# bravo1goingdark/ucfp

Measured on AMD Instinct MI355X. Metric: fingerprints/sec (batched ingest), higher is better.
Workload: dtype u8; 1 GPU; image multi (pHash+dHash+aHash bundle, 536 B/frame), 100000 synthetic 512x512 GRAY8 frames per GPU resident in HBM (BASELINE.json configs[1]); frames_per_gpu=100000, width=512, height=512, pixfmt=gray8, algorithm=multi

## Files before the change

ucfp_amd/csrc/common.h:

```cpp
#pragma once
#include <hip/hip_runtime.h>
#include <stddef.h>
#include <stdint.h>

#include "../../include/ucfp_hip.h"

namespace ucfp {

int capi_fail(int code, const char* fmt, ...);
int ctx_device(const ucfp_ctx* ctx);
bool have_gfx950();

}

#define HIP_TRY(expr)                                                                                \
    do {                                                                                             \
        hipError_t e_ = (expr);                                                                      \
        if (e_ != hipSuccess)                                                                        \
            return ucfp::capi_fail(UCFP_E_INDEX, "%s failed: %s", #expr, hipGetErrorString(e_));     \
    } while (0)

namespace ucfp {

struct DevArr {
// ... 94 lines not shown
int launch_png_decode(const uint8_t* png, const uint64_t* offsets, size_t n, uint32_t w, uint32_t h, int pixfmt, uint8_t* ws,
                      const PngWs& l, uint8_t* frames, size_t row_stride, size_t frame_stride, int32_t* status,
                      hipStream_t stream, hipStream_t side = nullptr, hipEvent_t fork = nullptr, hipEvent_t join = nullptr);
int launch_png_merge_status(const uint8_t* ws, const PngWs& l, size_t n, uint8_t* out, uint32_t rec, int32_t* status,
                            hipStream_t stream, const UpItem* d_items = nullptr);
size_t png_ragged_ws_bytes(size_t n, size_t png_bytes, size_t raw_total, PngWs* ws);
size_t png_raw_bytes(uint32_t w, uint32_t h, int pixfmt);
int launch_png_decode_ragged(const uint8_t* png, const uint64_t* offsets, const UpItem* d_items, size_t n, const uint32_t max_w[3],
                             uint8_t* ws, const PngWs& l, uint8_t* frames, int32_t* status, hipStream_t stream);

struct JpegWs {
    size_t clean = 0, info = 0, seg = 0, qtab = 0, coef = 0, coef_stride = 0, total = 0;
    size_t jpg_bytes = 0;
    uint32_t bxp = 0, byp = 0, max_seg = 0;
};
size_t jpeg_ws_bytes(size_t n, size_t jpg_bytes, uint32_t w, uint32_t h, JpegWs* ws);
int launch_jpeg_decode(const uint8_t* jpg, const uint64_t* offsets, size_t n, uint32_t w, uint32_t h, uint8_t* ws,
                       const JpegWs& l, uint8_t* frames, size_t row_stride, size_t frame_stride, int32_t* status,
                       hipStream_t stream);
int launch_jpeg_merge_status(const uint8_t* ws, const JpegWs& l, size_t n, uint8_t* out, uint32_t rec, int32_t* status,
                             hipStream_t stream, const UpItem* d_items = nullptr);
void jpeg_plane_geometry(uint32_t w, uint32_t h, uint32_t* bxp, uint32_t* byp, uint32_t* max_seg);
size_t jpeg_ragged_ws_bytes(size_t n, size_t jpg_bytes, size_t seg_words, size_t coef_words, JpegWs* ws);
int launch_jpeg_decode_ragged(const uint8_t* jpg, const uint64_t* offsets, const UpItem* d_items, size_t n, const uint32_t* d_first,
                              size_t idct_groups, uint8_t* ws, const JpegWs& l, uint8_t* frames, int32_t* status, hipStream_t stream);

struct HammingPlan {
    uint32_t qgroups = 0;
    int cap = 24;
    size_t sample_n = 0;
    uint32_t sample_parts = 0;
    size_t per_part = 0;
    size_t robust_n = 0;
    uint32_t slices = 0;
    size_t per_slice = 0;
    bool bound = false;
    size_t bound_n = 0;
    bool fast = false;
    uint32_t nstages = 0;
    size_t stage_end[12] = {0};
    uint32_t cand_cap = 0;
    uint32_t log_cap = 0;
    uint32_t fb_slices = 0;
    size_t fb_per_slice = 0;
};
constexpr uint32_t kHammingMaxBatch = 4096;
HammingPlan hamming_plan(size_t n, uint32_t nq, uint32_t k);
size_t hamming_workspace_bytes(const HammingPlan& p, uint32_t nq, uint32_t k);
int launch_hamming_search(const uint64_t* codes, const uint64_t* ids, size_t n,
                          const uint64_t* queries, uint32_t nq, uint32_t k, uint8_t* ws,
                          const HammingPlan& p, uint64_t* out_ids, uint32_t* out_dist,
                          float* out_scores, uint32_t* out_cnt, hipStream_t stream,
                          const uint32_t* ids_ascending = nullptr);
int launch_ids_order_update(const uint64_t* ids, size_t n, bool first, uint32_t* state, hipStream_t stream);
int launch_hamming_scores(const uint32_t* dist, size_t total, float* scores, hipStream_t stream);

constexpr uint32_t kHammingDirectMaxQ = 8, kHammingDirectMaxK = 32, kHammingDirectZeroBytes = 12288;
bool hamming_direct_ok(size_t n, uint32_t nq, uint32_t k);
size_t hamming_direct_state_bytes();
int launch_hamming_direct(const uint64_t* codes, const uint64_t* ids, size_t n, const uint64_t* queries, uint32_t nq,
                          uint32_t k, uint8_t* state, uint64_t* out_ids, uint32_t* out_dist, float* out_scores,
                          uint32_t* out_cnt, hipStream_t stream, const uint32_t* ids_ascending = nullptr);

struct SelectPlan {
    uint32_t slices = 0;
    size_t per_slice = 0;
};
SelectPlan select_plan(size_t n, uint32_t nq);
bool select_pruned_ok(size_t n, uint32_t nq, uint32_t k);
size_t select_pruned_ws_bytes(size_t n, uint32_t nq);
int launch_select_pruned_u32(const uint32_t* keys, const uint64_t* ids, size_t n, uint32_t nq, uint32_t k, uint32_t* mins,
                             uint64_t* out_ids, uint32_t* out_key, uint32_t* out_cnt, hipStream_t stream,
                             const uint32_t* run_flag);
int launch_select_topk_u32(const uint32_t* keys, const uint64_t* ids, size_t n, const SelectPlan& p,
                           uint32_t nq, uint32_t k, uint64_t* part_ids, uint32_t* part_key,
                           uint32_t* part_cnt, hipStream_t stream, const uint32_t* run_flag = nullptr);
int launch_topk_select_lists_u32(const uint64_t* base_ids, const uint32_t* base_key, const uint32_t* ckey,
                                 const uint32_t* crow, const uint32_t* ccnt, uint32_t cap, const uint64_t* ids,
                                 uint32_t nq, uint32_t k, uint64_t* out_ids, uint32_t* out_key, uint32_t* out_cnt,
                                 uint32_t* overflow, hipStream_t stream);
struct CosinePrunePlan {
    uint32_t cs_shift = 5;
    uint32_t qpad = 16;
    uint32_t nchunks = 0;
    uint32_t waves = 0;
    uint32_t capq = 32;
};
constexpr uint32_t kPruneCand = 2048;
bool cosine_prune_ok(const float* rows, uint32_t dim, const float* queries, uint32_t nq_pass, size_t n, uint32_t k);
CosinePrunePlan cosine_prune_plan(size_t n, uint32_t nq_pass, uint32_t k, bool approx = false);
float cosine_mins_eps(uint32_t dim);
uint32_t cosine_list_queries(uint32_t dim);
bool cosine_mins_f16_ok(const float* rows, uint32_t dim, const float* queries, uint32_t nq_pass, size_t n, uint32_t k);
int launch_cosine_norms_image(const float* queries, size_t nq, uint32_t dim, float* norms, void* image, uint32_t* zero2,
                              hipStream_t stream);
int launch_cosine_mins_f16(const float* rows, const float* norms, size_t n, uint32_t dim, const void* image, const float* qnorm,
                           uint32_t nq_pass, const CosinePrunePlan& p, uint32_t* mins, uint32_t* wmin, uint32_t* flag,
                           hipStream_t stream);
int launch_cosine_keys_dense_mfma(const float* rows, const float* norms, size_t n, uint32_t dim, const float* queries,
                                  const float* qnorm, uint32_t nq_pass, uint32_t* keys, const uint32_t* run_flag,
                                  hipStream_t stream);
int launch_cosine_keys_mins(const float* rows, const float* norms, size_t n, uint32_t dim, const float* queries,
                            const float* qnorm, uint32_t nq_pass, const CosinePrunePlan& p, uint32_t* mins, uint32_t* wmin,
                            hipStream_t stream);
int launch_cosine_keys_list(const float* rows, const float* norms, size_t n, uint32_t dim, const float* queries,
                            const float* qnorm, uint32_t nq_pass, const CosinePrunePlan& p, const void* list,
                            const uint32_t* nlist, uint32_t* ckeys, const uint32_t* fallback_flag, hipStream_t stream);
// ... 191 lines not shown
```

ucfp_amd/csrc/hamming.hip:

```cpp

#include <hip/hip_runtime.h>
#include <math.h>
#include <stdint.h>
#include <stdlib.h>

#include "common.h"

namespace ucfp {

constexpr int kWave = 64;
constexpr uint32_t kSub = 8;

__device__ __forceinline__ uint32_t hamming64(uint64_t q, uint64_t x) {
    const uint32_t lo = (uint32_t)q ^ (uint32_t)x;
    const uint32_t hi = (uint32_t)(q >> 32) ^ (uint32_t)(x >> 32);
    return __builtin_popcount(hi) + __builtin_popcount(lo);
}

__global__ __launch_bounds__(256) void hamming_sample_hist(const uint64_t* __restrict__ codes,
                                                           size_t sample_n, size_t per_part,
                                                           const uint64_t* __restrict__ queries,
                                                           uint32_t nq, uint32_t* __restrict__ hist) {
    __shared__ uint32_t h[65 * kWave];
    const int lane = threadIdx.x & 63, wave = threadIdx.x >> 6;
// ... 982 lines not shown
                bi = oi;
            }
        }
        if (bd == 0xffffffffu) break;
        if (lane == 0) {
            out_ids[(size_t)q * k + r] = bi;
            out_d[(size_t)q * k + r] = bd;
        }
        ld = bd;
        li = bi;
        first = false;
        emitted++;
    }
    if (lane == 0) {
        for (uint32_t r = emitted; r < k; r++) {
            out_ids[(size_t)q * k + r] = ~0ull;
            out_d[(size_t)q * k + r] = 0xffffffffu;
        }
        out_cnt[q] = emitted;
    }
}

__global__ void hamming_reset_lists(uint32_t nq, uint32_t* __restrict__ cand_cnt, uint32_t* __restrict__ overflow) {
    const uint32_t q = blockIdx.x * blockDim.x + threadIdx.x;
    if (q == 0) *overflow = 0;
    if (q < nq)
        for (uint32_t u = 0; u < kSub; u++) cand_cnt[(size_t)q * kSub + u] = 0;
}

__global__ void hamming_scores(const uint32_t* __restrict__ dist, size_t total, float* __restrict__ scores) {
    const size_t i = (size_t)blockIdx.x * blockDim.x + threadIdx.x;
    if (i < total) {
        const uint32_t d = dist[i];
        scores[i] = d == 0xffffffffu ? -1.0f : 1.0f - (float)d * (1.0f / 64.0f);
    }
}


namespace {
void slice_range(size_t n, uint32_t qgroups, uint32_t want_waves, size_t min_per_slice, uint32_t& slices,
                 size_t& per_slice) {
    uint32_t s = (want_waves + qgroups - 1) / (qgroups ? qgroups : 1);
    const size_t max_s = (n + min_per_slice - 1) / min_per_slice;
    if (s > max_s) s = (uint32_t)(max_s ? max_s : 1);
    if (s < 1) s = 1;
    if (s > 8192) s = 8192;
    per_slice = (n + s - 1) / s;
    per_slice = (per_slice + 31) & ~(size_t)31;
    slices = (uint32_t)((n + per_slice - 1) / (per_slice ? per_slice : 1));
    if (slices < 1) slices = 1;
}
}

__global__ void ids_order_update_kernel(const uint64_t* __restrict__ ids, size_t n, bool first, uint32_t* __restrict__ state) {
    const size_t i = (size_t)blockIdx.x * blockDim.x + threadIdx.x;
    if (i >= n) return;
    uint64_t* last = reinterpret_cast<uint64_t*>(state + 2);
    bool ok;
    if (i == 0) ok = first || ids[0] > *last;
    else ok = ids[i] > ids[i - 1];
    if (!ok) state[0] = 0;
}
__global__ void ids_order_last_kernel(const uint64_t* __restrict__ ids, size_t n, uint32_t* __restrict__ state) {
    *reinterpret_cast<uint64_t*>(state + 2) = ids[n - 1];
}
int launch_ids_order_update(const uint64_t* ids, size_t n, bool first, uint32_t* state, hipStream_t stream) {
    if (n == 0) return 0;
    hipLaunchKernelGGL(ids_order_update_kernel, dim3((unsigned)((n + 255) / 256)), dim3(256), 0, stream, ids, n, first, state);
    hipLaunchKernelGGL(ids_order_last_kernel, dim3(1), dim3(1), 0, stream, ids, n, state);
    return 0;
}

static bool few_queries(size_t n, uint32_t nq);
constexpr uint32_t kBoundGroups = 256;
constexpr size_t kBoundCodes = (size_t)1 << 18;

HammingPlan hamming_plan(size_t n, uint32_t nq, uint32_t k) {
    HammingPlan p;
    p.qgroups = (nq + kWave - 1) / kWave;
    p.cap = k <= 16 ? 24 : k <= 40 ? 64 : 160;
    if (n == 0) return p;
    size_t s = 32768;
    if (s > n) s = n;
    p.sample_n = s;
    p.sample_parts = (uint32_t)((s + 1023) / 1024);
    p.per_part = (s + p.sample_parts - 1) / p.sample_parts;
    p.fast = n >= (size_t)1 << 18 && n - 1 <= 0xfffffff0u;
    p.robust_n = n;
    p.bound = p.fast && !few_queries(n, nq) && k <= 64 && !getenv("UCFP_HAMMING_NO_BOUND");
    const bool short_chain = p.bound && nq <= 256 && k <= 16;
    if (p.bound) {
        size_t bc = short_chain ? (size_t)1 << 20 : kBoundCodes;
        static const char* bl = getenv("UCFP_HAMMING_BOUND_LOG2_SMALL");
        if (bl && nq <= 256) bc = (size_t)1 << atoi(bl);
        static const char* bg = getenv("UCFP_HAMMING_BOUND_LOG2_LARGE");
        if (bg && nq > 256) bc = (size_t)1 << atoi(bg);
        p.bound_n = (n < bc ? n : bc) & ~(size_t)(128 - 1);
    }
    if (p.fast) {
        size_t e = p.bound ? p.bound_n : p.sample_n;
        size_t growth = short_chain ? 64 : nq <= 256 ? 8 : 4;
        static const char* gs = getenv("UCFP_HAMMING_GROWTH_SMALL");
        if (gs && nq <= 256) growth = (size_t)atoi(gs);
        static const char* gl = getenv("UCFP_HAMMING_GROWTH_LARGE");
        if (gl && nq > 256) growth = (size_t)atoi(gl);
        static const char* nomerge = getenv("UCFP_HAMMING_NO_STAGE_MERGE");
        do {
            e = e * growth < n ? e * growth : n;
            if (!nomerge && n - e < e / 4) e = n;
            p.stage_end[p.nstages++] = e;
        } while (e < n && p.nstages < 12);
        p.stage_end[p.nstages - 1] = n;
        p.robust_n = 0;
        size_t cc = (size_t)k * growth * 5 * p.nstages * 2;
        if (cc < 2048) cc = 2048;
        if (cc > 65536) cc = 65536;
        cc = (cc + 63) & ~(size_t)63;
        p.cand_cap = (uint32_t)cc;
        p.log_cap = 1024;
        slice_range(n, p.qgroups, 256 * 16, 4096, p.fb_slices, p.fb_per_slice);
        return p;
    }
// ... 175 lines not shown
```

ucfp_amd/csrc/index.hip:

```cpp

#include <hip/hip_runtime.h>

#include <cstdarg>
#include <cstdio>
#include <cstdlib>
#include <cstring>
#include <map>
#include <mutex>
#include <new>
#include <unordered_map>
#include <vector>

#include "../../include/ucfp_hip.h"
#include "common.h"

using ucfp::capi_fail;

namespace {

struct DevBuf {
    uint8_t* p = nullptr;
    size_t cap = 0;
    int ensure(size_t need) {
        if (cap >= need) return 0;
        if (p) (void)hipFree(p);
        p = nullptr;
        cap = 0;
        const size_t want = need + need / 4 + 4096;
        HIP_TRY(hipMalloc((void**)&p, want));
        cap = want;
        return 0;
    }
    void release() {
        if (p) (void)hipFree(p);
        p = nullptr;
        cap = 0;
    }
};

struct Shard {
    uint64_t* ids = nullptr;
    uint8_t* rows = nullptr;
    float* norms = nullptr;
    size_t n = 0, cap = 0;
    std::unordered_map<uint64_t, size_t> pos;
    std::vector<uint64_t> host_ids;
    uint32_t* order = nullptr;
};

__global__ void scatter_rows_kernel(const uint64_t* __restrict__ src_ids, const uint8_t* __restrict__ src_rows,
                                    const uint64_t* __restrict__ dst_row, size_t n, size_t row_bytes,
                                    uint64_t* __restrict__ ids, uint8_t* __restrict__ rows) {
    const size_t i = blockIdx.x;
    if (i >= n) return;
    const size_t r = dst_row[i];
    if (threadIdx.x == 0) ids[r] = src_ids[i];
    const uint32_t* s = reinterpret_cast<const uint32_t*>(src_rows + i * row_bytes);
    uint32_t* d = reinterpret_cast<uint32_t*>(rows + r * row_bytes);
    for (size_t w = threadIdx.x; w < row_bytes / 4; w += blockDim.x) d[w] = s[w];
}

__global__ void gather_norms_kernel(const float* __restrict__ src, const uint64_t* __restrict__ dst_row, size_t n,
                                    float* __restrict__ norms) {
    const size_t i = (size_t)blockIdx.x * blockDim.x + threadIdx.x;
    if (i < n) norms[dst_row[i]] = src[i];
}

int ensure_order_state(Shard& s, hipStream_t st) {
    if (s.order) return 0;
    if (hipMalloc((void**)&s.order, 16) != hipSuccess) return -1;
    static const uint32_t init[4] = {1u, 0u, 0u, 0u};
    if (hipMemcpyAsync(s.order, init, 16, hipMemcpyHostToDevice, st) != hipSuccess) return -1;
    return 0;
}

}

struct ucfp_index {
    ucfp_ctx* ctx = nullptr;
    int device = 0;
    int kind = 0;
    uint32_t dim = 0;
    uint32_t flags = 0;
    size_t row_bytes = 0;
    std::mutex mu;
    std::map<uint32_t, Shard> shards;
    hipStream_t stream = nullptr;
    DevBuf ws_slot[2];
    DevBuf direct_state[2];
    hipEvent_t ws_done[2] = {nullptr, nullptr};
    unsigned ws_next = 0, ws_cur = 0;
    hipEvent_t data_ready = nullptr;
    DevBuf stage;
};

namespace ucfp {
int index_kind(const ucfp_index* ix) { return ix->kind; }
int index_device(const ucfp_index* ix) { return ix->device; }
uint32_t index_dim(const ucfp_index* ix) { return ix->dim; }
}

namespace {

int shard_reserve(ucfp_index* ix, Shard& s, size_t need, hipStream_t st) {
    if (need <= s.cap) return 0;
    size_t ncap = s.cap ? s.cap * 2 : 1024;
    while (ncap < need) ncap *= 2;
    uint64_t* nids = nullptr;
    uint8_t* nrows = nullptr;
    float* nnorms = nullptr;
    HIP_TRY(hipMalloc((void**)&nids, ncap * 8));
    HIP_TRY(hipMalloc((void**)&nrows, ncap * ix->row_bytes));
    if (ix->kind == UCFP_INDEX_COSINE_F32) HIP_TRY(hipMalloc((void**)&nnorms, ncap * 4));
    if (s.n) {
        HIP_TRY(hipMemcpyAsync(nids, s.ids, s.n * 8, hipMemcpyDeviceToDevice, st));
        HIP_TRY(hipMemcpyAsync(nrows, s.rows, s.n * ix->row_bytes, hipMemcpyDeviceToDevice, st));
        if (nnorms) HIP_TRY(hipMemcpyAsync(nnorms, s.norms, s.n * 4, hipMemcpyDeviceToDevice, st));
    }
    HIP_TRY(hipStreamSynchronize(st));
    if (s.ids) (void)hipFree(s.ids);
    if (s.rows) (void)hipFree(s.rows);
    if (s.norms) (void)hipFree(s.norms);
    s.ids = nids;
    s.rows = nrows;
    s.norms = nnorms;
    s.cap = ncap;
    return 0;
}

size_t align256(size_t x) { return (x + 255) & ~(size_t)255; }

int search_shard_dev(ucfp_index* ix, const Shard* s, const void* d_queries, size_t nq, uint32_t k,
                     uint64_t* d_out_ids, float* d_out_scores, uint32_t* d_out_keys, uint32_t* d_out_cnt,
                     hipStream_t st) {
    const size_t n = s ? s->n : 0;
    if (ix->kind == UCFP_INDEX_HAMMING64 && nq <= ucfp::kHammingDirectMaxQ && ucfp::hamming_direct_ok(n, (uint32_t)nq, k) &&
        !getenv("UCFP_HAMMING_NO_DIRECT")) {
        DevBuf& stt = ix->direct_state[ix->ws_cur];
        if (!stt.p) {
            int rc = stt.ensure(ucfp::hamming_direct_state_bytes());
            if (rc) return rc;
            HIP_TRY(hipMemsetAsync(stt.p, 0, ucfp::kHammingDirectZeroBytes, st));
        }
        uint32_t* keys = d_out_keys;
        if (!keys) {
            int rc = ix->ws_slot[ix->ws_cur].ensure(nq * k * 4 + 256);
            if (rc) return rc;
            keys = reinterpret_cast<uint32_t*>(ix->ws_slot[ix->ws_cur].p);
        }
        ucfp::launch_hamming_direct(reinterpret_cast<const uint64_t*>(s->rows), s->ids, n,
                                    reinterpret_cast<const uint64_t*>(d_queries), (uint32_t)nq, k, stt.p, d_out_ids, keys,
                                    d_out_scores, d_out_cnt, st, s->order);
        HIP_TRY(hipGetLastError());
        return 0;
    }
    if (ix->kind == UCFP_INDEX_HAMMING64) {
        const size_t chunk = nq < ucfp::kHammingMaxBatch ? nq : ucfp::kHammingMaxBatch;
        ucfp::HammingPlan p = ucfp::hamming_plan(n, (uint32_t)chunk, k);
        size_t need = ucfp::hamming_workspace_bytes(p, (uint32_t)chunk, k) + 4096;
        if (nq % chunk) {
            const uint32_t tail = (uint32_t)(nq % chunk);
            const size_t nt = ucfp::hamming_workspace_bytes(ucfp::hamming_plan(n, tail, k), tail, k) + 4096;
            need = nt > need ? nt : need;
        }
        uint32_t* keys = d_out_keys;
        size_t keys_off = 0;
        if (!keys) {
            keys_off = align256(need);
            need = keys_off + nq * k * 4;
        }
        int rc = ix->ws_slot[ix->ws_cur].ensure(need);
        if (rc) return rc;
        if (!keys) keys = reinterpret_cast<uint32_t*>(ix->ws_slot[ix->ws_cur].p + keys_off);
        const uint64_t* dq = reinterpret_cast<const uint64_t*>(d_queries);
        for (size_t c0 = 0; c0 < nq; c0 += chunk) {
            const uint32_t cn = (uint32_t)(nq - c0 < chunk ? nq - c0 : chunk);
            if (cn != chunk) p = ucfp::hamming_plan(n, cn, k);
            ucfp::launch_hamming_search(s ? reinterpret_cast<const uint64_t*>(s->rows) : nullptr, s ? s->ids : nullptr,
                                        n, dq + c0, cn, k, ix->ws_slot[ix->ws_cur].p, p, d_out_ids + c0 * k, keys + c0 * k,
                                        d_out_scores ? d_out_scores + c0 * k : nullptr, d_out_cnt + c0, st,
// ... 226 lines not shown
    HIP_TRY(hipGetLastError());
    return 0;
}

int check_search_args(ucfp_index* ix, const void* q, size_t nq, uint32_t k, const void* ids, const void* cnt) {
    if (!ix) return capi_fail(UCFP_E_INVALID, "index is NULL");
    if (k > UCFP_INDEX_MAX_K) return capi_fail(UCFP_E_INVALID, "k = %u exceeds UCFP_INDEX_MAX_K = %u", k, UCFP_INDEX_MAX_K);
    if (nq && k && (!q || !ids || !cnt)) return capi_fail(UCFP_E_INVALID, "queries/out_ids/out_counts is NULL");
    if (nq > 4000000u) return capi_fail(UCFP_E_INVALID, "query batch %zu too large for one call (max 4 000 000)", nq);
    return 0;
}

}

extern "C" {

int ucfp_index_create(ucfp_ctx* ctx, int kind, uint32_t dim, uint32_t flags, ucfp_index** out) {
    if (!ctx || !out) return capi_fail(UCFP_E_INVALID, "ctx/out is NULL");
    *out = nullptr;
    if (kind != UCFP_INDEX_HAMMING64 && kind != UCFP_INDEX_COSINE_F32)
        return capi_fail(UCFP_E_UNSUPPORTED, "unknown index kind %d", kind);
    if (kind == UCFP_INDEX_COSINE_F32 && (dim == 0 || dim > 65536))
        return capi_fail(UCFP_E_INVALID, "cosine index needs 1 <= dim <= 65536 (got %u)", dim);
    ucfp_index* ix = new (std::nothrow) ucfp_index();
    if (!ix) return capi_fail(UCFP_E_INDEX, "out of host memory");
    ix->ctx = ctx;
    ix->device = ucfp::ctx_device(ctx);
    ix->kind = kind;
    ix->dim = kind == UCFP_INDEX_HAMMING64 ? 1 : dim;
    ix->flags = flags;
    ix->row_bytes = kind == UCFP_INDEX_HAMMING64 ? 8 : (size_t)dim * 4;
    hipError_t e = hipSetDevice(ix->device);
    if (e == hipSuccess) e = hipStreamCreateWithFlags(&ix->stream, hipStreamNonBlocking);
    for (int i = 0; i < 2 && e == hipSuccess; i++) e = hipEventCreateWithFlags(&ix->ws_done[i], hipEventDisableTiming);
    if (e == hipSuccess) e = hipEventCreateWithFlags(&ix->data_ready, hipEventDisableTiming);
    if (e != hipSuccess) {
        delete ix;
        return capi_fail(UCFP_E_INDEX, "index stream creation failed: %s", hipGetErrorString(e));
    }
    *out = ix;
    return UCFP_OK;
}

void ucfp_index_destroy(ucfp_index* ix) {
    if (!ix) return;
    (void)hipSetDevice(ix->device);
    (void)hipDeviceSynchronize();
    for (auto& kv : ix->shards) {
        if (kv.second.ids) (void)hipFree(kv.second.ids);
        if (kv.second.rows) (void)hipFree(kv.second.rows);
        if (kv.second.norms) (void)hipFree(kv.second.norms);
        if (kv.second.order) (void)hipFree(kv.second.order);
    }
    for (auto& w : ix->ws_slot) w.release();
    for (auto& w : ix->direct_state) w.release();
    ix->stage.release();
    if (ix->stream) (void)hipStreamDestroy(ix->stream);
    for (hipEvent_t ev : ix->ws_done)
        if (ev) (void)hipEventDestroy(ev);
    if (ix->data_ready) (void)hipEventDestroy(ix->data_ready);
    delete ix;
}

int ucfp_index_upsert(ucfp_index* ix, uint32_t tenant, const uint64_t* ids, const void* rows, size_t n) {
    if (!ix) return capi_fail(UCFP_E_INVALID, "index is NULL");
    if (n == 0) return UCFP_OK;
    if (!ids || !rows) return capi_fail(UCFP_E_INVALID, "ids/rows is NULL");
    std::lock_guard<std::mutex> lk(ix->mu);
    HIP_TRY(hipSetDevice(ix->device));
    Shard& s = ix->shards[tenant];
    hipStream_t st = ix->stream;
    for (hipEvent_t ev : ix->ws_done) HIP_TRY(hipStreamWaitEvent(st, ev, 0));
    HIP_TRY(hipStreamWaitEvent(st, ix->data_ready, 0));
    const bool mapped = !(ix->flags & UCFP_INDEX_APPEND_ONLY);
    std::vector<uint64_t> dst(n);
    std::vector<uint8_t> keep(n, 1);
    size_t new_n = s.n;
    if (mapped) {
        std::unordered_map<uint64_t, size_t> last;
        last.reserve(n * 2);
        for (size_t i = 0; i < n; i++) last[ids[i]] = i;
        for (size_t i = 0; i < n; i++) {
            if (last[ids[i]] != i) {
                keep[i] = 0;
                continue;
            }
            auto it = s.pos.find(ids[i]);
            if (it != s.pos.end()) dst[i] = it->second;
            else dst[i] = new_n++;
        }
    } else {
        for (size_t i = 0; i < n; i++) dst[i] = new_n++;
    }
    int rc = shard_reserve(ix, s, new_n, st);
    if (rc) return rc;
    size_t m = 0;
    for (size_t i = 0; i < n; i++) m += keep[i];
    const size_t o_ids = 0, o_dst = align256(m * 8), o_rows = align256(o_dst + m * 8);
    const size_t o_norm = align256(o_rows + m * ix->row_bytes);
    rc = ix->stage.ensure(o_norm + m * 4 + 256);
    if (rc) return rc;
    std::vector<uint64_t> h_ids(m), h_dst(m);
    std::vector<uint8_t> h_rows(m * ix->row_bytes);
    size_t j = 0;
    for (size_t i = 0; i < n; i++) {
        if (!keep[i]) continue;
        h_ids[j] = ids[i];
        h_dst[j] = dst[i];
        memcpy(h_rows.data() + j * ix->row_bytes, (const uint8_t*)rows + i * ix->row_bytes, ix->row_bytes);
        j++;
    }
    uint8_t* sp = ix->stage.p;
    HIP_TRY(hipMemcpyAsync(sp + o_ids, h_ids.data(), m * 8, hipMemcpyHostToDevice, st));
    HIP_TRY(hipMemcpyAsync(sp + o_dst, h_dst.data(), m * 8, hipMemcpyHostToDevice, st));
    HIP_TRY(hipMemcpyAsync(sp + o_rows, h_rows.data(), m * ix->row_bytes, hipMemcpyHostToDevice, st));
    hipLaunchKernelGGL(scatter_rows_kernel, dim3((unsigned)m), dim3(64), 0, st,
                       reinterpret_cast<const uint64_t*>(sp + o_ids), sp + o_rows,
                       reinterpret_cast<const uint64_t*>(sp + o_dst), m, ix->row_bytes, s.ids, s.rows);
    if (ix->kind == UCFP_INDEX_COSINE_F32) {
        ucfp::launch_cosine_norms(reinterpret_cast<const float*>(sp + o_rows), m, ix->dim,
                                  reinterpret_cast<float*>(sp + o_norm), st);
        hipLaunchKernelGGL(gather_norms_kernel, dim3((unsigned)((m + 255) / 256)), dim3(256), 0, st,
                           reinterpret_cast<const float*>(sp + o_norm), reinterpret_cast<const uint64_t*>(sp + o_dst),
                           m, s.norms);
    }
    if (!mapped && ix->kind == UCFP_INDEX_HAMMING64 && m) {
        if (ensure_order_state(s, st)) return capi_fail(UCFP_E_INDEX, "out of device memory");
        ucfp::launch_ids_order_update(s.ids + s.n, m, s.n == 0, s.order, st);
    }
    HIP_TRY(hipGetLastError());
    HIP_TRY(hipEventRecord(ix->data_ready, st));
    HIP_TRY(hipStreamSynchronize(st));
    if (mapped) {
        s.host_ids.resize(new_n);
        for (size_t t = 0; t < m; t++) {
            s.pos[h_ids[t]] = h_dst[t];
            s.host_ids[h_dst[t]] = h_ids[t];
        }
    }
    s.n = new_n;
    return UCFP_OK;
}

int ucfp_index_append_dev(ucfp_index* ix, uint32_t tenant, const uint64_t* d_ids, const void* d_rows, size_t n,
                          void* stream) {
    if (!ix) return capi_fail(UCFP_E_INVALID, "index is NULL");
    if (!(ix->flags & UCFP_INDEX_APPEND_ONLY))
        return capi_fail(UCFP_E_UNSUPPORTED, "append_dev needs an index created with UCFP_INDEX_APPEND_ONLY");
    if (n == 0) return UCFP_OK;
    if (!d_ids || !d_rows) return capi_fail(UCFP_E_INVALID, "ids/rows is NULL");
    std::lock_guard<std::mutex> lk(ix->mu);
    HIP_TRY(hipSetDevice(ix->device));
    Shard& s = ix->shards[tenant];
    hipStream_t st = (hipStream_t)stream;
    for (hipEvent_t ev : ix->ws_done) HIP_TRY(hipStreamWaitEvent(st, ev, 0));
    HIP_TRY(hipStreamWaitEvent(st, ix->data_ready, 0));
    int rc = shard_reserve(ix, s, s.n + n, st);
    if (rc) return rc;
    HIP_TRY(hipMemcpyAsync(s.ids + s.n, d_ids, n * 8, hipMemcpyDeviceToDevice, st));
    HIP_TRY(hipMemcpyAsync(s.rows + s.n * ix->row_bytes, d_rows, n * ix->row_bytes, hipMemcpyDeviceToDevice, st));
    if (ix->kind == UCFP_INDEX_HAMMING64) {
        if (ensure_order_state(s, st)) return capi_fail(UCFP_E_INDEX, "out of device memory");
        ucfp::launch_ids_order_update(s.ids + s.n, n, s.n == 0, s.order, st);
    }
    if (ix->kind == UCFP_INDEX_COSINE_F32)
        ucfp::launch_cosine_norms(reinterpret_cast<const float*>(s.rows + s.n * ix->row_bytes), n, ix->dim,
                                  s.norms + s.n, st);
    HIP_TRY(hipGetLastError());
    HIP_TRY(hipEventRecord(ix->data_ready, st));
    s.n += n;
    return UCFP_OK;
}

int ucfp_index_delete(ucfp_index* ix, uint32_t tenant, const uint64_t* ids, size_t n, size_t* n_removed) {
    if (n_removed) *n_removed = 0;
    if (!ix) return capi_fail(UCFP_E_INVALID, "index is NULL");
    if (ix->flags & UCFP_INDEX_APPEND_ONLY)
        return capi_fail(UCFP_E_UNSUPPORTED, "delete on an APPEND_ONLY index");
    if (n && !ids) return capi_fail(UCFP_E_INVALID, "ids is NULL");
    std::lock_guard<std::mutex> lk(ix->mu);
    auto sit = ix->shards.find(tenant);
    if (sit == ix->shards.end()) return UCFP_OK;
    Shard& s = sit->second;
    HIP_TRY(hipSetDevice(ix->device));
    hipStream_t st = ix->stream;
    for (hipEvent_t ev : ix->ws_done) HIP_TRY(hipStreamWaitEvent(st, ev, 0));
    HIP_TRY(hipStreamWaitEvent(st, ix->data_ready, 0));
    size_t removed = 0;
    for (size_t i = 0; i < n; i++) {
        auto it = s.pos.find(ids[i]);
        if (it == s.pos.end()) continue;
        const size_t r = it->second, last = s.n - 1;
        if (r != last) {
            HIP_TRY(hipMemcpyAsync(s.ids + r, s.ids + last, 8, hipMemcpyDeviceToDevice, st));
            HIP_TRY(hipMemcpyAsync(s.rows + r * ix->row_bytes, s.rows + last * ix->row_bytes, ix->row_bytes,
                                   hipMemcpyDeviceToDevice, st));
            if (s.norms) HIP_TRY(hipMemcpyAsync(s.norms + r, s.norms + last, 4, hipMemcpyDeviceToDevice, st));
            const uint64_t moved = s.host_ids[last];
            s.host_ids[r] = moved;
            s.pos[moved] = r;
        }
        s.pos.erase(it);
        s.host_ids.pop_back();
        s.n--;
        removed++;
    }
    HIP_TRY(hipEventRecord(ix->data_ready, st));
    HIP_TRY(hipStreamSynchronize(st));
    if (n_removed) *n_removed = removed;
    return UCFP_OK;
}

int ucfp_index_size(ucfp_index* ix, uint32_t tenant, size_t* out) {
    if (!ix || !out) return capi_fail(UCFP_E_INVALID, "index/out is NULL");
    std::lock_guard<std::mutex> lk(ix->mu);
    auto it = ix->shards.find(tenant);
    *out = it == ix->shards.end() ? 0 : it->second.n;
    return UCFP_OK;
}

int ucfp_index_flush(ucfp_index* ix) {
    if (!ix) return capi_fail(UCFP_E_INVALID, "index is NULL");
    std::lock_guard<std::mutex> lk(ix->mu);
    HIP_TRY(hipSetDevice(ix->device));
    HIP_TRY(hipDeviceSynchronize());
    return UCFP_OK;
}

int ucfp_index_save(ucfp_index* ix, const char* path) {
    if (!ix || !path) return capi_fail(UCFP_E_INVALID, "index/path is NULL");
    std::lock_guard<std::mutex> lk(ix->mu);
    HIP_TRY(hipSetDevice(ix->device));
    HIP_TRY(hipDeviceSynchronize());
    FILE* f = fopen(path, "wb");
    if (!f) return capi_fail(UCFP_E_INDEX, "cannot open %s for writing", path);
    bool ok = fwrite("UCFPIDX1", 1, 8, f) == 8;
    const uint32_t hdr[2] = {(uint32_t)ix->kind, ix->dim};
    const uint64_t rb = ix->row_bytes;
    uint32_t nt[2] = {0, 0};
    for (auto& kv : ix->shards) nt[0] += kv.second.n ? 1u : 0u;
    ok = ok && fwrite(hdr, 4, 2, f) == 2 && fwrite(&rb, 8, 1, f) == 1 && fwrite(nt, 4, 2, f) == 2;
    std::vector<uint8_t> host;
    const size_t chunk_rows = 1u << 20;
    for (auto& kv : ix->shards) {
        const Shard& s = kv.second;
        if (!s.n || !ok) continue;
        const uint32_t th[2] = {kv.first, 0};
        const uint64_t n = s.n;
        ok = ok && fwrite(th, 4, 2, f) == 2 && fwrite(&n, 8, 1, f) == 1;
        for (int pass = 0; pass < 2 && ok; pass++) {
            const size_t unit = pass == 0 ? 8 : ix->row_bytes;
            const uint8_t* src = pass == 0 ? reinterpret_cast<const uint8_t*>(s.ids) : s.rows;
            for (size_t r0 = 0; r0 < s.n && ok; r0 += chunk_rows) {
                const size_t cnt = s.n - r0 < chunk_rows ? s.n - r0 : chunk_rows;
                host.resize(cnt * unit);
                if (hipMemcpy(host.data(), src + r0 * unit, cnt * unit, hipMemcpyDeviceToHost) != hipSuccess) ok = false;
                ok = ok && fwrite(host.data(), 1, cnt * unit, f) == cnt * unit;
            }
        }
    }
    ok = (fclose(f) == 0) && ok;
// ... 54 lines not shown
    HIP_TRY(hipSetDevice(ix->device));
    hipStream_t st = (hipStream_t)stream;
    if (k == 0) {
        HIP_TRY(hipMemsetAsync(d_out_counts, 0, nq * 4, st));
        return UCFP_OK;
    }
    auto it = ix->shards.find(tenant);
    const Shard* s = it == ix->shards.end() ? nullptr : &it->second;
    ix->ws_cur = ix->kind == UCFP_INDEX_HAMMING64 ? (ix->ws_next++ & 1u) : 0u;
    HIP_TRY(hipStreamWaitEvent(st, ix->ws_done[ix->ws_cur], 0));
    HIP_TRY(hipStreamWaitEvent(st, ix->data_ready, 0));
    rc = search_shard_dev(ix, s, d_queries, nq, k, d_out_ids, d_out_scores, d_out_dist, d_out_counts, st);
    HIP_TRY(hipEventRecord(ix->ws_done[ix->ws_cur], st));
    return rc;
}

int ucfp_index_search(ucfp_index* ix, uint32_t tenant, const void* queries, size_t nq, uint32_t k,
                      uint64_t* out_ids, float* out_scores, uint32_t* out_dist, uint32_t* out_counts) {
    int rc = check_search_args(ix, queries, nq, k, out_ids, out_counts);
    if (rc) return rc;
    if (nq == 0) return UCFP_OK;
    if (k == 0) {
        memset(out_counts, 0, nq * 4);
        return UCFP_OK;
    }
    const size_t qbytes = nq * ix->row_bytes;
    const size_t o_q = 0, o_ids = align256(qbytes), o_sc = align256(o_ids + nq * k * 8);
    const size_t o_d = align256(o_sc + nq * k * 4), o_c = align256(o_d + nq * k * 4);
    const size_t total = align256(o_c + nq * 4);
    hipStream_t st;
    uint8_t* buf = nullptr;
    {
        std::lock_guard<std::mutex> lk(ix->mu);
        HIP_TRY(hipSetDevice(ix->device));
        st = ix->stream;
        HIP_TRY(hipMalloc((void**)&buf, total));
    }
    hipError_t e = hipMemcpyAsync(buf + o_q, queries, qbytes, hipMemcpyHostToDevice, st);
    if (e == hipSuccess) {
        rc = ucfp_index_search_dev(ix, tenant, buf + o_q, nq, k, reinterpret_cast<uint64_t*>(buf + o_ids),
                                   reinterpret_cast<float*>(buf + o_sc), reinterpret_cast<uint32_t*>(buf + o_d),
                                   reinterpret_cast<uint32_t*>(buf + o_c), st);
        if (rc == 0) {
            e = hipMemcpyAsync(out_ids, buf + o_ids, nq * k * 8, hipMemcpyDeviceToHost, st);
            if (e == hipSuccess && out_scores)
                e = hipMemcpyAsync(out_scores, buf + o_sc, nq * k * 4, hipMemcpyDeviceToHost, st);
            if (e == hipSuccess && out_dist)
                e = hipMemcpyAsync(out_dist, buf + o_d, nq * k * 4, hipMemcpyDeviceToHost, st);
            if (e == hipSuccess) e = hipMemcpyAsync(out_counts, buf + o_c, nq * 4, hipMemcpyDeviceToHost, st);
        }
    }
    hipError_t e2 = hipStreamSynchronize(st);
    (void)hipFree(buf);
    if (rc) return rc;
    if (e != hipSuccess) return capi_fail(UCFP_E_INDEX, "search copy failed: %s", hipGetErrorString(e));
    if (e2 != hipSuccess) return capi_fail(UCFP_E_INDEX, "search failed: %s", hipGetErrorString(e2));
    return UCFP_OK;
}

int ucfp_topk_merge_dev(ucfp_ctx* ctx, int kind, const uint64_t* d_part_ids, const uint32_t* d_part_keys,
                        uint32_t parts, size_t nq, uint32_t k, uint64_t* d_out_ids, float* d_out_scores,
                        uint32_t* d_out_keys, uint32_t* d_out_counts, void* stream) {
    if (!ctx) return capi_fail(UCFP_E_INVALID, "ctx is NULL");
    if (kind != UCFP_INDEX_HAMMING64 && kind != UCFP_INDEX_COSINE_F32)
        return capi_fail(UCFP_E_UNSUPPORTED, "unknown index kind %d", kind);
    if (nq == 0 || k == 0) return UCFP_OK;
    if (!d_part_ids || !d_part_keys || !d_out_ids || !d_out_keys || !d_out_counts)
        return capi_fail(UCFP_E_INVALID, "merge buffers must not be NULL");
    if (k > UCFP_INDEX_MAX_K) return capi_fail(UCFP_E_INVALID, "k too large");
    hipStream_t st = (hipStream_t)stream;
    ucfp::launch_topk_merge_u32(d_part_ids, d_part_keys, parts, (uint32_t)nq, k, d_out_ids, d_out_keys, d_out_counts,
                                nullptr, st);
    if (d_out_scores) {
        if (kind == UCFP_INDEX_HAMMING64) ucfp::launch_hamming_scores(d_out_keys, nq * k, d_out_scores, st);
        else ucfp::launch_cosine_scores_from_keys(d_out_keys, nq * k, d_out_scores, st);
    }
    HIP_TRY(hipGetLastError());
    return UCFP_OK;
}

}
```

Before: 26.11 million fingerprints/s.

## Fuse hamming append copy with order check and defer freeing grown shard buffers

Replaces the two device-to-device memcpys, the order-check kernel and the separate last-id kernel with one append kernel that copies ids and codes while checking ascending order, using a double-buffered last-id slot. Shard growth no longer synchronizes the stream before freeing the old buffers; old buffers go to an event-guarded retire list swept later. This cuts launches and host syncs on the ingest/add path, at the cost of holding old allocations in memory longer and more bookkeeping complexity.

```diff
diff --git a/ucfp_amd/csrc/common.h b/ucfp_amd/csrc/common.h
--- a/ucfp_amd/csrc/common.h
+++ b/ucfp_amd/csrc/common.h
@@ -170,7 +170,9 @@
                           const HammingPlan& p, uint64_t* out_ids, uint32_t* out_dist,
                           float* out_scores, uint32_t* out_cnt, hipStream_t stream,
                           const uint32_t* ids_ascending = nullptr);
-int launch_ids_order_update(const uint64_t* ids, size_t n, bool first, uint32_t* state, hipStream_t stream);
+int launch_ids_order_update(const uint64_t* ids, size_t n, bool first, uint32_t* state, uint32_t slot, hipStream_t stream);
+int launch_hamming_append(const uint64_t* ids, const uint64_t* codes, size_t n, bool first, uint64_t* dst_ids,
+                          uint64_t* dst_codes, uint32_t* state, uint32_t slot, hipStream_t stream);
 int launch_hamming_scores(const uint32_t* dist, size_t total, float* scores, hipStream_t stream);
 
 constexpr uint32_t kHammingDirectMaxQ = 8, kHammingDirectMaxK = 32, kHammingDirectZeroBytes = 12288;
diff --git a/ucfp_amd/csrc/hamming.hip b/ucfp_amd/csrc/hamming.hip
--- a/ucfp_amd/csrc/hamming.hip
+++ b/ucfp_amd/csrc/hamming.hip
@@ -1058,22 +1058,35 @@
 }
 }
 
-__global__ void ids_order_update_kernel(const uint64_t* __restrict__ ids, size_t n, bool first, uint32_t* __restrict__ state) {
+template <bool kCopy>
+__global__ void hamming_append_kernel(const uint64_t* __restrict__ ids, const uint64_t* __restrict__ codes, size_t n, bool first,
+                                      uint32_t slot, uint64_t* __restrict__ dst_ids, uint64_t* __restrict__ dst_codes,
+                                      uint32_t* __restrict__ state) {
     const size_t i = (size_t)blockIdx.x * blockDim.x + threadIdx.x;
     if (i >= n) return;
     uint64_t* last = reinterpret_cast<uint64_t*>(state + 2);
+    const uint64_t id = ids[i];
     bool ok;
-    if (i == 0) ok = first || ids[0] > *last;
-    else ok = ids[i] > ids[i - 1];
+    if (i == 0) ok = first || id > last[slot];
+    else ok = id > ids[i - 1];
     if (!ok) state[0] = 0;
-}
-__global__ void ids_order_last_kernel(const uint64_t* __restrict__ ids, size_t n, uint32_t* __restrict__ state) {
-    *reinterpret_cast<uint64_t*>(state + 2) = ids[n - 1];
-}
-int launch_ids_order_update(const uint64_t* ids, size_t n, bool first, uint32_t* state, hipStream_t stream) {
+    if (kCopy) {
+        dst_ids[i] = id;
+        dst_codes[i] = codes[i];
+    }
+    if (i == n - 1) last[slot ^ 1u] = id;
+}
+int launch_ids_order_update(const uint64_t* ids, size_t n, bool first, uint32_t* state, uint32_t slot, hipStream_t stream) {
     if (n == 0) return 0;
-    hipLaunchKernelGGL(ids_order_update_kernel, dim3((unsigned)((n + 255) / 256)), dim3(256), 0, stream, ids, n, first, state);
-    hipLaunchKernelGGL(ids_order_last_kernel, dim3(1), dim3(1), 0, stream, ids, n, state);
+    hipLaunchKernelGGL(hamming_append_kernel<false>, dim3((unsigned)((n + 255) / 256)), dim3(256), 0, stream, ids, nullptr, n,
+                       first, slot, nullptr, nullptr, state);
+    return 0;
+}
+int launch_hamming_append(const uint64_t* ids, const uint64_t* codes, size_t n, bool first, uint64_t* dst_ids,
+                          uint64_t* dst_codes, uint32_t* state, uint32_t slot, hipStream_t stream) {
+    if (n == 0) return 0;
+    hipLaunchKernelGGL(hamming_append_kernel<true>, dim3((unsigned)((n + 255) / 256)), dim3(256), 0, stream, ids, codes, n,
+                       first, slot, dst_ids, dst_codes, state);
     return 0;
 }
 
diff --git a/ucfp_amd/csrc/index.hip b/ucfp_amd/csrc/index.hip
--- a/ucfp_amd/csrc/index.hip
+++ b/ucfp_amd/csrc/index.hip
@@ -13,6 +13,7 @@
 
 #include "../../include/ucfp_hip.h"
 #include "common.h"
+#include "shard_buffers.h"
 
 using ucfp::capi_fail;
 
@@ -46,6 +47,30 @@
     std::unordered_map<uint64_t, size_t> pos;
     std::vector<uint64_t> host_ids;
     uint32_t* order = nullptr;
+    uint32_t order_slot = 0;
+};
+
+struct HipShardBackend {
+    using Event = hipEvent_t;
+    hipStream_t st;
+    void* alloc(size_t bytes) {
+        void* p = nullptr;
+        if (hipMalloc(&p, bytes) == hipSuccess) return p;
+        (void)hipGetLastError();
+        return nullptr;
+    }
+    void free(void* p) { (void)hipFree(p); }
+    bool copy(void* dst, const void* src, size_t bytes) {
+        return hipMemcpyAsync(dst, src, bytes, hipMemcpyDeviceToDevice, st) == hipSuccess;
+    }
+    bool record(Event* ev) {
+        if (hipEventCreateWithFlags(ev, hipEventDisableTiming) != hipSuccess) return false;
+        if (hipEventRecord(*ev, st) == hipSuccess) return true;
+        (void)hipEventDestroy(*ev);
+        return false;
+    }
+    bool query(Event ev) { return hipEventQuery(ev) == hipSuccess; }
+    void drop(Event ev) { (void)hipEventDestroy(ev); }
 };
 
 __global__ void scatter_rows_kernel(const uint64_t* __restrict__ src_ids, const uint8_t* __restrict__ src_rows,
@@ -68,9 +93,9 @@
 
 int ensure_order_state(Shard& s, hipStream_t st) {
     if (s.order) return 0;
-    if (hipMalloc((void**)&s.order, 16) != hipSuccess) return -1;
-    static const uint32_t init[4] = {1u, 0u, 0u, 0u};
-    if (hipMemcpyAsync(s.order, init, 16, hipMemcpyHostToDevice, st) != hipSuccess) return -1;
+    if (hipMalloc((void**)&s.order, 32) != hipSuccess) return -1;
+    if (hipMemsetD32Async(reinterpret_cast<hipDeviceptr_t>(s.order), 1, 8, st) != hipSuccess) return -1;
+    s.order_slot = 0;
     return 0;
 }
 
@@ -92,6 +117,7 @@
     unsigned ws_next = 0, ws_cur = 0;
     hipEvent_t data_ready = nullptr;
     DevBuf stage;
+    ucfp::shardbuf::RetireList<HipShardBackend> retired;
 };
 
 namespace ucfp {
@@ -104,28 +130,33 @@
 
 int shard_reserve(ucfp_index* ix, Shard& s, size_t need, hipStream_t st) {
     if (need <= s.cap) return 0;
-    size_t ncap = s.cap ? s.cap * 2 : 1024;
-    while (ncap < need) ncap *= 2;
-    uint64_t* nids = nullptr;
-    uint8_t* nrows = nullptr;
-    float* nnorms = nullptr;
-    HIP_TRY(hipMalloc((void**)&nids, ncap * 8));
-    HIP_TRY(hipMalloc((void**)&nrows, ncap * ix->row_bytes));
-    if (ix->kind == UCFP_INDEX_COSINE_F32) HIP_TRY(hipMalloc((void**)&nnorms, ncap * 4));
-    if (s.n) {
-        HIP_TRY(hipMemcpyAsync(nids, s.ids, s.n * 8, hipMemcpyDeviceToDevice, st));
-        HIP_TRY(hipMemcpyAsync(nrows, s.rows, s.n * ix->row_bytes, hipMemcpyDeviceToDevice, st));
-        if (nnorms) HIP_TRY(hipMemcpyAsync(nnorms, s.norms, s.n * 4, hipMemcpyDeviceToDevice, st));
-    }
-    HIP_TRY(hipStreamSynchronize(st));
-    if (s.ids) (void)hipFree(s.ids);
-    if (s.rows) (void)hipFree(s.rows);
-    if (s.norms) (void)hipFree(s.norms);
-    s.ids = nids;
-    s.rows = nrows;
-    s.norms = nnorms;
-    s.cap = ncap;
+    namespace sb = ucfp::shardbuf;
+    HipShardBackend be{st};
+    sb::Buffers b;
+    b.p[0] = s.ids;
+    b.p[1] = s.rows;
+    b.p[2] = s.norms;
+    b.cap = s.cap;
+    sb::Layout lay;
+    lay.unit[0] = 8;
+    lay.unit[1] = ix->row_bytes;
+    lay.unit[2] = ix->kind == UCFP_INDEX_COSINE_F32 ? 4 : 0;
+    const int rc = sb::reserve(be, ix->retired, b, lay, s.n, need);
+    const size_t ncap = sb::grown_capacity(s.cap, need);
+    if (rc == sb::kNoMemory) return capi_fail(UCFP_E_INDEX, "out of device memory growing a shard to %zu rows", ncap);
+    if (rc)
+        return capi_fail(UCFP_E_INDEX, "growing a shard to %zu rows failed: %s", ncap, hipGetErrorString(hipGetLastError()));
+    s.ids = static_cast<uint64_t*>(b.p[0]);
+    s.rows = static_cast<uint8_t*>(b.p[1]);
+    s.norms = static_cast<float*>(b.p[2]);
+    s.cap = b.cap;
     return 0;
+}
+
+void sweep_retired(ucfp_index* ix) {
+    if (ix->retired.entries.empty()) return;
+    HipShardBackend be{nullptr};
+    ix->retired.sweep(be);
 }
 
 size_t align256(size_t x) { return (x + 255) & ~(size_t)255; }
@@ -458,6 +489,8 @@
         if (kv.second.norms) (void)hipFree(kv.second.norms);
         if (kv.second.order) (void)hipFree(kv.second.order);
     }
+    HipShardBackend be{nullptr};
+    ix->retired.free_all(be);
     for (auto& w : ix->ws_slot) w.release();
     for (auto& w : ix->direct_state) w.release();
     ix->stage.release();
@@ -532,11 +565,13 @@
     }
     if (!mapped && ix->kind == UCFP_INDEX_HAMMING64 && m) {
         if (ensure_order_state(s, st)) return capi_fail(UCFP_E_INDEX, "out of device memory");
-        ucfp::launch_ids_order_update(s.ids + s.n, m, s.n == 0, s.order, st);
+        ucfp::launch_ids_order_update(s.ids + s.n, m, s.n == 0, s.order, s.order_slot, st);
     }
     HIP_TRY(hipGetLastError());
     HIP_TRY(hipEventRecord(ix->data_ready, st));
     HIP_TRY(hipStreamSynchronize(st));
+    if (!mapped && ix->kind == UCFP_INDEX_HAMMING64 && m) s.order_slot ^= 1u;
+    sweep_retired(ix);
     if (mapped) {
         s.host_ids.resize(new_n);
         for (size_t t = 0; t < m; t++) {
@@ -563,17 +598,19 @@
     HIP_TRY(hipStreamWaitEvent(st, ix->data_ready, 0));
     int rc = shard_reserve(ix, s, s.n + n, st);
     if (rc) return rc;
-    HIP_TRY(hipMemcpyAsync(s.ids + s.n, d_ids, n * 8, hipMemcpyDeviceToDevice, st));
-    HIP_TRY(hipMemcpyAsync(s.rows + s.n * ix->row_bytes, d_rows, n * ix->row_bytes, hipMemcpyDeviceToDevice, st));
     if (ix->kind == UCFP_INDEX_HAMMING64) {
         if (ensure_order_state(s, st)) return capi_fail(UCFP_E_INDEX, "out of device memory");
-        ucfp::launch_ids_order_update(s.ids + s.n, n, s.n == 0, s.order, st);
-    }
-    if (ix->kind == UCFP_INDEX_COSINE_F32)
+        ucfp::launch_hamming_append(d_ids, reinterpret_cast<const uint64_t*>(d_rows), n, s.n == 0, s.ids + s.n,
+                                    reinterpret_cast<uint64_t*>(s.rows) + s.n, s.order, s.order_slot, st);
+    } else {
+        HIP_TRY(hipMemcpyAsync(s.ids + s.n, d_ids, n * 8, hipMemcpyDeviceToDevice, st));
+        HIP_TRY(hipMemcpyAsync(s.rows + s.n * ix->row_bytes, d_rows, n * ix->row_bytes, hipMemcpyDeviceToDevice, st));
         ucfp::launch_cosine_norms(reinterpret_cast<const float*>(s.rows + s.n * ix->row_bytes), n, ix->dim,
                                   s.norms + s.n, st);
+    }
     HIP_TRY(hipGetLastError());
     HIP_TRY(hipEventRecord(ix->data_ready, st));
+    if (ix->kind == UCFP_INDEX_HAMMING64) s.order_slot ^= 1u;
     s.n += n;
     return UCFP_OK;
 }
@@ -613,6 +650,7 @@
     }
     HIP_TRY(hipEventRecord(ix->data_ready, st));
     HIP_TRY(hipStreamSynchronize(st));
+    sweep_retired(ix);
     if (n_removed) *n_removed = removed;
     return UCFP_OK;
 }
@@ -773,6 +811,10 @@
     }
     hipError_t e2 = hipStreamSynchronize(st);
     (void)hipFree(buf);
+    {
+        std::lock_guard<std::mutex> lk(ix->mu);
+        sweep_retired(ix);
+    }
     if (rc) return rc;
     if (e != hipSuccess) return capi_fail(UCFP_E_INDEX, "search copy failed: %s", hipGetErrorString(e));
     if (e2 != hipSuccess) return capi_fail(UCFP_E_INDEX, "search failed: %s", hipGetErrorString(e2));
diff --git a/ucfp_amd/csrc/shard_buffers.h b/ucfp_amd/csrc/shard_buffers.h
--- /dev/null
+++ b/ucfp_amd/csrc/shard_buffers.h
@@ -0,0 +1,103 @@
+#pragma once
+#include <cstddef>
+#include <cstdint>
+#include <vector>
+
+namespace ucfp {
+namespace shardbuf {
+
+constexpr int kMaxBufs = 3;
+constexpr size_t kFirstCap = 1024;
+
+enum { kOk = 0, kNoMemory = 1, kBackendFailed = 2 };
+
+struct Buffers {
+    void* p[kMaxBufs] = {nullptr, nullptr, nullptr};
+    size_t cap = 0;
+};
+
+struct Layout {
+    size_t unit[kMaxBufs] = {0, 0, 0};
+    size_t row_bytes() const { return unit[0] + unit[1] + unit[2]; }
+};
+
+inline size_t grown_capacity(size_t cap, size_t need) {
+    size_t ncap = cap ? cap * 2 : kFirstCap;
+    while (ncap < need) ncap *= 2;
+    return ncap;
+}
+
+template <class B>
+struct RetireList {
+    struct Entry {
+        void* p[kMaxBufs];
+        size_t bytes;
+        typename B::Event ev;
+    };
+    std::vector<Entry> entries;
+    size_t bytes = 0;
+
+    size_t sweep(B& b) {
+        size_t freed = 0, kept = 0;
+        for (size_t i = 0; i < entries.size(); i++) {
+            Entry& e = entries[i];
+            if (!b.query(e.ev)) {
+                entries[kept++] = e;
+                continue;
+            }
+            release(b, e);
+            freed += e.bytes;
+        }
+        entries.resize(kept);
+        bytes -= freed;
+        return freed;
+    }
+
+    void free_all(B& b) {
+        for (Entry& e : entries) release(b, e);
+        entries.clear();
+        bytes = 0;
+    }
+
+  private:
+    static void release(B& b, Entry& e) {
+        for (void* q : e.p)
+            if (q) b.free(q);
+        b.drop(e.ev);
+    }
+};
+
+template <class B>
+int reserve(B& b, RetireList<B>& retired, Buffers& s, const Layout& lay, size_t live, size_t need) {
+    if (need <= s.cap) return kOk;
+    const size_t ncap = grown_capacity(s.cap, need);
+    void* np[kMaxBufs] = {nullptr, nullptr, nullptr};
+    auto undo = [&](int rc) {
+        for (void* q : np)
+            if (q) b.free(q);
+        return rc;
+    };
+    for (int i = 0; i < kMaxBufs; i++) {
+        if (!lay.unit[i]) continue;
+        np[i] = b.alloc(ncap * lay.unit[i]);
+        if (!np[i]) return undo(kNoMemory);
+    }
+    if (s.cap) {
+        retired.entries.reserve(retired.entries.size() + 1);
+        if (live)
+            for (int i = 0; i < kMaxBufs; i++)
+                if (np[i] && !b.copy(np[i], s.p[i], live * lay.unit[i])) return undo(kBackendFailed);
+        typename RetireList<B>::Entry e;
+        if (!b.record(&e.ev)) return undo(kBackendFailed);
+        for (int i = 0; i < kMaxBufs; i++) e.p[i] = s.p[i];
+        e.bytes = s.cap * lay.row_bytes();
+        retired.entries.push_back(e);
+        retired.bytes += e.bytes;
+    }
+    for (int i = 0; i < kMaxBufs; i++) s.p[i] = np[i];
+    s.cap = ncap;
+    return kOk;
+}
+
+}
+}
```

Result: no change. 26.07 million fingerprints/s (-0.1%).
